# danielreardon/scintools

Hardware: NVIDIA H100
Metric: theta-theta eta-trials/sec on 4096x8192 dynspec (higher is better)
Workload: dtype f32

## Files before the change

### scintools_b200/csrc/thth.cu

```cuda
#include <float.h>
#include <limits.h>
#include <math.h>
#include <stdlib.h>

#include <type_traits>

#include "bf16_pack.cuh"
#include "lanczos.cuh"
#include "thth.cuh"
#include "tma.cuh"

namespace sb {

#ifndef SB_HOST_EMU
int eig_cluster_launch(const float2* d_M, int ld, int n_max, const int* d_nred, int e0,
                       int nb, double* d_eigs, int* d_status, int* d_iters, double tol,
                       double etol, int max_iter, cudaStream_t st);

int eig_half_launch(const float2* d_M, const unsigned* d_Mb, int ld, const int* d_nred, int e0,
                    int nb, double* d_eigs, int* d_status, int* d_iters, double tol, double etol,
                    int max_iter, bool tensor, cudaStream_t st);

#endif

enum { ST_OK = 0, ST_INDEX_ERROR = 1, ST_ZERO_START = 2, ST_TOO_SMALL = 4,
       ST_NOT_CONVERGED = 8 };

__global__ void thth_prep_kernel(ThthGeom g, const double* __restrict__ etas,
                                 int neta, int ld, int* __restrict__ idx,
                                 int* __restrict__ nred) {
    int e = blockIdx.x;
    if (e >= neta) return;
    double eta = etas[e];
    int lane = threadIdx.x;
    int base = 0;
    int* out = idx + (size_t)e * ld;
    for (int k0 = 0; k0 < g.n; k0 += 32) {
        int k = k0 + lane;
        bool keep = false;
        if (k < g.n) {
            double t = g.th[k];
            keep = (__dmul_rn(__dmul_rn(t, t), eta) < g.tau_absmax) &&
                   (fabs(t) < g.fd_half);
        }
        unsigned m = __ballot_sync(0xffffffffu, keep);
        if (keep) out[base + __popc(m & ((1u << lane) - 1u))] = k;
        base += __popc(m);
    }
    if (lane == 0) nred[e] = base;
}

__global__ void thth_indexerr_kernel(ThthGeom g, const double* __restrict__ etas,
                                     int* __restrict__ status) {
    int e = blockIdx.y;
    double eta = etas[e];
    long long total = (long long)g.n * g.n;
    bool bad = false;
    for (long long p = (long long)blockIdx.x * blockDim.x + threadIdx.x;
         p < total; p += (long long)gridDim.x * blockDim.x) {
        int i = (int)(p / g.n), j = (int)(p % g.n);
        ThthPoint pt = thth_point(g, eta, g.th[j], g.th[i]);
        bad |= pt.index_error;
    }
    if (__any_sync(0xffffffffu, bad) && (threadIdx.x & 31) == 0)
        atomicOr(status + e, ST_INDEX_ERROR);
}

#define SB_BUILD_EB 8

__device__ __forceinline__ unsigned pack_f16x2(float2 v) {
#ifdef SB_HOST_EMU
    const __half2 h = __floats2half2_rn(v.x, v.y);
    return (unsigned)h.x | ((unsigned)h.y << 16);
#else
    unsigned r;
    asm("cvt.rn.f16x2.f32 %0, %1, %2;" : "=r"(r) : "f"(v.y), "f"(v.x));
    return r;
#endif
}

__global__ void cs_absmax_kernel(const float2* __restrict__ cs, long long rows, long long ncols,
                                 long long pitch, unsigned* __restrict__ out) {
    float m = 0.f;
    const long long per_row4 = ncols >> 1;
    const long long total = rows * per_row4;
    for (long long i = (long long)blockIdx.x * blockDim.x + threadIdx.x; i < total;
         i += (long long)gridDim.x * blockDim.x) {
        const long long r = i / per_row4, c = i - r * per_row4;
        const float4 q = __ldg(reinterpret_cast<const float4*>(cs + r * pitch) + c);
        m = fmaxf(fmaxf(fmaxf(fabsf(q.x), fabsf(q.y)), fmaxf(fabsf(q.z), fabsf(q.w))), m);
    }
    if (ncols & 1) {
        for (long long r = (long long)blockIdx.x * blockDim.x + threadIdx.x; r < rows;
             r += (long long)gridDim.x * blockDim.x) {
            const float2 q = __ldg(cs + r * pitch + ncols - 1);
            m = fmaxf(fmaxf(fabsf(q.x), fabsf(q.y)), m);
        }
    }
    if (!(m == m)) m = 3.0e38f;
    m = fminf(m, 3.0e38f);
#pragma unroll
    for (int o = 16; o > 0; o >>= 1) m = fmaxf(m, __shfl_xor_sync(0xffffffffu, m, o));
    if ((threadIdx.x & 31) == 0) atomicMax(out, __float_as_uint(m));
}

template <int PACK, int ROWS, typename OFF>
__global__ void __launch_bounds__(32 * (32 / ROWS), ROWS == 8 ? 5 : 3)
thth_build_kernel(ThthGeom g, const double* __restrict__ etas, int eta0, int nbatch,
                  int ld, const int* __restrict__ idx,
                  const int* __restrict__ nred, float2* __restrict__ M,
                  unsigned* __restrict__ Mb, const unsigned* __restrict__ absmax, float span) {
    constexpr int TY = 32 / ROWS;
    int p = blockIdx.y, ta = 0;
    const int T = ld / 32;
    while (p >= T - ta) { p -= T - ta; ++ta; }
    const int tb = ta + p;
    const int tx = threadIdx.x, ty = threadIdx.y;
    const int b = tb * 32 + tx;
    const double ntau_d = (double)g.ntau;
    const long long hfd = g.nfd / 2;
    int cj = -2;
    double thj = 0.0;
    int ci[ROWS];
    double dk[ROWS];
    int col[ROWS];
    unsigned conj = 0u;
    float wk[ROWS];
#pragma unroll
    for (int k = 0; k < ROWS; ++k) { ci[k] = -2; dk[k] = 0.0; col[k] = -1; wk[k] = 0.f; }
    const int e_end = min(nbatch, (int)(blockIdx.x + 1) * SB_BUILD_EB);
    __shared__ float s_hscale[SB_BUILD_EB];
    if (PACK != 0) {
        const int lin = ty * 32 + tx;
        if (lin < SB_BUILD_EB) {
            const int e = blockIdx.x * SB_BUILD_EB + lin;
            float hs = 1.f;
            if (e < e_end) {
                const float seta = sqrtf((float)(2.0 * etas[eta0 + e]));
                const float bound = __uint_as_float(*absmax) * seta * sqrtf(span);
                if (bound > 0.f && bound < 3.0e38f) {
                    const float q = 32768.f / bound;
                    hs = q >= 1.1754944e-38f ? __uint_as_float(__float_as_uint(q) & 0x7f800000u) : 1.1754944e-38f;
                }
            }
            s_hscale[lin] = hs;
        }
        __syncthreads();
    }
    const unsigned foff0 = (unsigned)(ta * 32 + ty) * (unsigned)ld + (unsigned)b;
    const unsigned frow = (unsigned)TY * (unsigned)ld;
    const unsigned woff0 = ((unsigned)(2 * ta) * (unsigned)(ld >> 3) + (unsigned)(b >> 3)) * 128u +
                           (unsigned)ty * 8u;
    for (int e = blockIdx.x * SB_BUILD_EB; e < e_end; ++e) {
        const int n = nred[eta0 + e];
        if (tb * 32 >= n) continue;
        const double eta = etas[eta0 + e];
        const int* id = idx + (size_t)(eta0 + e) * ld;
        const int j = b < n ? id[b] : -1;
        if (j != cj) {
            cj = j;
            thj = j >= 0 ? g.th[j] : 0.0;
#pragma unroll
            for (int k = 0; k < ROWS; ++k) ci[k] = -2;
        }
        const float seta = sqrtf((float)(2.0 * eta));
        float2* Me = M + (size_t)e * ld * ld;
        const float hscale = PACK != 0 ? s_hscale[e - blockIdx.x * SB_BUILD_EB] : 1.f;
        OFF off[ROWS];
        unsigned hit = 0u;
#pragma unroll
        for (int k = 0; k < ROWS; ++k) {
            const int la = ty + TY * k;
            off[k] = 0;
            if (ta == tb && tx < la) continue;
            const int a = ta * 32 + la;
            const int i = a < n ? id[a] : -1;
            if (i != ci[k]) {
                ci[k] = i;
                col[k] = -1;
                conj &= ~(1u << k);
                wk[k] = 0.f;
                dk[k] = 0.0;
                if (i >= 0 && j > i && i + j != g.n - 1) {
                    const double th1 = thj, th2 = g.th[i];
                    dk[k] = __dsub_rn(__dmul_rn(th1, th1), __dmul_rn(th2, th2));
                    const double bb = __dadd_rn(__dsub_rn(__dsub_rn(th1, th2), g.fd0), g.half_dfd);
                    const double fqd = floor_div_fast(bb, g.dfd, g.inv_dfd);
                    const long long fq = (fqd == fqd && fabs(fqd) < 9.0e18) ? (long long)fqd : LLONG_MIN;
                    wk[k] = sqrtf((float)fabs(th2 - th1));
                    if (fq < g.nfd && !(fq < -g.nfd)) {
                        const long long fi = fq < 0 ? fq + g.nfd : fq;
                        if (!g.cs_half) col[k] = (int)fi;
                        else if (fi >= hfd) col[k] = (int)(fi - hfd);
                        else if (fi == 0) col[k] = (int)hfd;
                        else { col[k] = (int)(hfd - fi); conj |= 1u << k; }
                    }
                }
            }
            if (col[k] >= 0) {
                const double aa = __dadd_rn(__dsub_rn(__dmul_rn(eta, dk[k]), g.tau0), g.half_dtau);
                const double tqd = floor_div_fast(aa, g.dtau, g.inv_dtau);
                if (tqd > 0.0 && tqd < ntau_d) {
                    const int tq = (int)tqd;
                    const int r = (conj >> k) & 1u ? (int)g.ntau - tq : tq;
                    off[k] = (OFF)r * (OFF)g.cs_pitch + (OFF)col[k];
                    hit |= 1u << k;
                }
            }
        }
        float2 val[ROWS];
#pragma unroll
        for (int k = 0; k < ROWS; ++k) val[k] = __ldg(g.cs + off[k]);
#pragma unroll
        for (int k = 0; k < ROWS; ++k) {
            const int la = ty + TY * k;
            const bool low = ta == tb && tx < la;
            float2 v = make_float2(0.f, 0.f);
            if (!low) {
                if (col[k] >= 0) {
                    if ((hit >> k) & 1u) {
                        v = val[k];
                        if ((conj >> k) & 1u) v.y = -v.y;
                        if (!g.coherent) v = make_float2(hypotf(v.x, v.y), 0.f);
                    }
                    const float wf = seta * wk[k];
                    v.x *= wf;
                    v.y *= wf;
                    if (!(fabsf(v.x) <= 3.402823466e+38f) || !(fabsf(v.y) <= 3.402823466e+38f)) {
                        v.x = nan_to_num(v.x);
                        v.y = nan_to_num(v.y);
                    }
                }
                const unsigned o = foff0 + (unsigned)k * frow;
                Me[o] = v;
                if (PACK == 1) Mb[(size_t)e * ld * ld + o] = pack_f16x2(make_float2(v.x * hscale, v.y * hscale));
            }
            if (PACK == 2) {
                const unsigned h = low ? 0u : pack_f16x2(make_float2(v.x * hscale, v.y * hscale));
                const int i8 = tx & 7, s0 = (tx & ~7) + 2 * (i8 & 3);
                const unsigned ha = __shfl_sync(0xffffffffu, h, s0);
                const unsigned hb = __shfl_sync(0xffffffffu, h, s0 + 1);
                const unsigned word = i8 < 4 ? ((ha & 0xffffu) | (hb << 16)) : ((ha >> 16) | (hb & 0xffff0000u));
                if (!(ta == tb && (tx >> 4) < (la >> 4))) {
                    unsigned* Mw = Mb + (size_t)e * ld * ld;
                    const unsigned swz = (unsigned)(((la & 15) >> 2) & 1) << 2;
                    Mw[woff0 + (unsigned)(la >> 4) * (unsigned)(ld >> 3) * 128u + (unsigned)((la & 15) - ty) * 8u +
                       ((unsigned)i8 ^ swz)] = word;
                }
            }
        }
    }
}

template <int THREADS, bool TMA, int NST, bool FAST = false>
__global__ void __launch_bounds__(THREADS)
thth_eig_kernel(const float2* __restrict__ Mbase, int ld,
                const int* __restrict__ nred, int eta0,
                double* __restrict__ eigs, int* __restrict__ status,
                int* __restrict__ iters, double tol, double etol, int max_iter, int nb) {
    extern __shared__ __align__(128) unsigned char smem_raw[];
    constexpr int NW = THREADS / 32;
    LanczosShared& S = *reinterpret_cast<LanczosShared*>(smem_raw);
    float2* v = reinterpret_cast<float2*>(smem_raw + sizeof(LanczosShared));
    float2* vp = v + ld;
    float2* w = vp + ld;
    float2* u = w + ld;
    float4* stages = reinterpret_cast<float4*>(u + ld);
    float2* part = reinterpret_cast<float2*>(stages);
    unsigned long long* mbar = reinterpret_cast<unsigned long long*>(
        reinterpret_cast<unsigned char*>(stages) +
        (TMA ? (size_t)NW * NST * 4096 : (size_t)NW * 4096));
    const int tid = threadIdx.x, lane = tid & 31, warp = tid >> 5;
    if (TMA) {
        if (tid == 0) {
            for (int i = 0; i < NW * NST; ++i) mbar_init(mbar + i, 1);
            fence_mbarrier_init();
        }
    }
    unsigned gi = 0, gc = 0;
    for (int e = blockIdx.x; e < nb; e += gridDim.x) {
    __syncthreads();
    const int n = nred[eta0 + e];
    const float2* M = Mbase + (size_t)e * ld * ld;
    const double qnan = __longlong_as_double(0x7ff8000000000000LL);

    if (status[eta0 + e] & ST_INDEX_ERROR) {
        if (tid == 0) { eigs[eta0 + e] = qnan; iters[eta0 + e] = 0; }
        continue;
    }
    if (n < 3) {
        if (tid == 0) {
            eigs[eta0 + e] = qnan; iters[eta0 + e] = 0;
            status[eta0 + e] |= ST_TOO_SMALL;
        }
        continue;
    }
    const int h = n / 2;
    double part0 = 0.0;
    for (int c = tid; c < ld; c += THREADS) {
        float2 x = make_float2(0.f, 0.f);
        if (c < n && c > h) x = M[(size_t)h * ld + c];
        else if (c < h) { x = M[(size_t)c * ld + h]; x.y = -x.y; }
        v[c] = x;
        vp[c] = make_float2(0.f, 0.f);
        part0 += (double)x.x * x.x + (double)x.y * x.y;
    }
    part0 = warp_sum(part0);
    if (lane == 0) S.red[0][warp] = part0;
    if (tid == 0) {
        S.done = 0; S.lo = 0.0; S.theta = 0.0; S.res = 0.0; S.m_lo2 = 0; S.lo2 = 0.0;
        S.next_check = 1; S.m_last = 0; S.beta2[0] = 0.0;
    }
    __syncthreads();
    double nrm2 = 0.0;
    for (int k = 0; k < NW; ++k) nrm2 += S.red[0][k];
    if (!(nrm2 > 0.0) || !isfinite(nrm2)) {
        if (tid == 0) {
            eigs[eta0 + e] = qnan; iters[eta0 + e] = 0;
            status[eta0 + e] |= ST_ZERO_START;
        }
        continue;
    }
    {
        float s = (float)(1.0 / sqrt(nrm2));
        for (int c = tid; c < ld; c += THREADS) { v[c].x *= s; v[c].y *= s; }
    }
    __syncthreads();

    const int ncol4 = (n + 1) >> 1;
    const int nchunk = (n + 511) / 512;
    float4* mystage = stages + (size_t)warp * NST * 256;
    unsigned long long* mybar = mbar + warp * NST;
    float beta_prev = 0.f;
    int m = 0;
    for (int it = 0; it < max_iter; ++it) {
        for (int c = tid; c < ld; c += THREADS) w[c] = make_float2(0.f, 0.f);
        __syncthreads();
        if constexpr (TMA) {
            float4 yc[8];
#pragma unroll
            for (int j = 0; j < 8; ++j) yc[j] = make_float4(0.f, 0.f, 0.f, 0.f);
            const int K = (n - 2 >= warp) ? (n - 2 - warp) / NW + 1 : 0;
            const bool tail = ncol4 < 256;
            const float4* v4 = reinterpret_cast<const float4*>(v);
            for (int k = 0; k < NST && k < K; ++k) {
                const int st = gi % NST;
                ++gi;
                if (lane == 0) {
                    const int a = warp + NW * k;
                    const int c_lo = (a + 1) & ~1;
                    const unsigned bytes = (unsigned)(2 * ncol4 - c_lo) * 8u;
                    mbar_expect_tx(mybar + st, bytes);
                    bulk_g2s(reinterpret_cast<float2*>(mystage + st * 256) + c_lo,
                             M + (size_t)a * ld + c_lo, bytes, mybar + st);
                }
            }
            int k = 0;
            auto run_rows = [&](auto JSc) {
                constexpr int JS = decltype(JSc)::value;
                for (; k < K && ((warp + NW * k + 1) >> 6) == JS; ++k) {
                    const int a = warp + NW * k;
                    const int first4 = (a + 1) >> 1;
                    const float2 xa = v[a];
                    const int st = gc % NST;
                    const unsigned par = (gc / NST) & 1u;
                    ++gc;
                    while (!mbar_try_wait(mybar + st, par)) {}
                    const float4* sg = mystage + st * 256;
                    float rxa = 0.f, rxb = 0.f, rya = 0.f, ryb = 0.f;
#pragma unroll
                    for (int j = JS; j < 8; ++j) {
                        const int c4 = lane + 32 * j;
                        float4 q = sg[c4];
                        bool ok = (j > JS) || (c4 >= first4);
                        if (tail) ok = ok && (c4 < ncol4);
                        if (!ok) q = make_float4(0.f, 0.f, 0.f, 0.f);
                        float4 x = make_float4(0.f, 0.f, 0.f, 0.f);
                        if (ok) x = v4[c4];
                        rxa = fmaf(q.x, x.x, rxa); rxb = fmaf(-q.y, x.y, rxb);
                        rxa = fmaf(q.z, x.z, rxa); rxb = fmaf(-q.w, x.w, rxb);
                        rya = fmaf(q.x, x.y, rya); ryb = fmaf(q.y, x.x, ryb);
                        rya = fmaf(q.z, x.w, rya); ryb = fmaf(q.w, x.z, ryb);
                        yc[j].x = fmaf(q.x, xa.x, yc[j].x); yc[j].x = fmaf(q.y, xa.y, yc[j].x);
                        yc[j].y = fmaf(q.x, xa.y, yc[j].y); yc[j].y = fmaf(-q.y, xa.x, yc[j].y);
                        yc[j].z = fmaf(q.z, xa.x, yc[j].z); yc[j].z = fmaf(q.w, xa.y, yc[j].z);
                        yc[j].w = fmaf(q.z, xa.y, yc[j].w); yc[j].w = fmaf(-q.w, xa.x, yc[j].w);
                    }
                    __syncwarp();
                    const bool more = k + NST < K;
                    const int st2 = gi % NST;
                    if (more) ++gi;
                    if (lane == 0 && more) {
                        const int a2 = warp + NW * (k + NST);
                        const int c_lo = (a2 + 1) & ~1;
                        const unsigned bytes = (unsigned)(2 * ncol4 - c_lo) * 8u;
                        mbar_expect_tx(mybar + st2, bytes);
                        bulk_g2s(reinterpret_cast<float2*>(mystage + st2 * 256) + c_lo,
                                 M + (size_t)a2 * ld + c_lo, bytes, mybar + st2);
                    }
                    const float rx = rxa + rxb, ry = rya + ryb;
                    const bool hi = lane & 16;
                    float keep = hi ? ry : rx;
                    keep += __shfl_xor_sync(0xffffffffu, hi ? rx : ry, 16);
                    keep += __shfl_xor_sync(0xffffffffu, keep, 8);
                    keep += __shfl_xor_sync(0xffffffffu, keep, 4);
                    keep += __shfl_xor_sync(0xffffffffu, keep, 2);
                    keep += __shfl_xor_sync(0xffffffffu, keep, 1);
                    if (lane == 0) w[a].x += keep;
                    if (lane == 16) w[a].y += keep;
                }
            };
            run_rows(std::integral_constant<int, 0>{});
            run_rows(std::integral_constant<int, 1>{});
            run_rows(std::integral_constant<int, 2>{});
            run_rows(std::integral_constant<int, 3>{});
            run_rows(std::integral_constant<int, 4>{});
            run_rows(std::integral_constant<int, 5>{});
            run_rows(std::integral_constant<int, 6>{});
            run_rows(std::integral_constant<int, 7>{});
            __syncthreads();
#pragma unroll
            for (int j = 0; j < 8; ++j)
                *reinterpret_cast<float4*>(part + warp * 512 + 2 * (lane + 32 * j)) = yc[j];
            __syncthreads();
            for (int c = tid; c < 512; c += THREADS) {
                float sx = 0.f, sy = 0.f;
#pragma unroll
                for (int kk = 0; kk < NW; ++kk) { sx += part[kk * 512 + c].x; sy += part[kk * 512 + c].y; }
                if (c < ld) u[c] = make_float2(sx, sy);
            }
            fence_proxy_async();
            __syncthreads();
        } else {
        for (int cb = 0; cb < nchunk; ++cb) {
            float4 yc[8];
#pragma unroll
            for (int j = 0; j < 8; ++j) yc[j] = make_float4(0.f, 0.f, 0.f, 0.f);
            const int chunk_end = min(n, (cb + 1) * 512);
            const int K = (chunk_end - 2 >= warp) ? (chunk_end - 2 - warp) / NW + 1 : 0;
            if (TMA) {
                for (int k = 0; k < NST && k < K; ++k) {
                    const int st = gi % NST;
                    ++gi;
                    if (lane == 0) {
                        const int a = warp + NW * k;
                        const int c_lo = (a + 1) & ~1;
                        const unsigned bytes = (unsigned)(2 * ncol4 - c_lo) * 8u;
                        mbar_expect_tx(mybar + st, bytes);
                        bulk_g2s(reinterpret_cast<float2*>(mystage + st * 256) + c_lo,
                                 M + (size_t)a * ld + c_lo, bytes, mybar + st);
                    }
                }
            }
            for (int k = 0; k < K; ++k) {
                const int a = warp + NW * k;
                const int first4 = (a + 1) >> 1;
                const float2 xa = v[a];
                float4 mm[8];
                if (TMA) {
                    const int st = gc % NST;
                    const unsigned par = (gc / NST) & 1u;
                    ++gc;
                    while (!mbar_try_wait(mybar + st, par)) {}
                    const float4* sg = mystage + st * 256;
                    const int jlo = max(0, (first4 - lane + 31) >> 5);
                    const int jhi = (ncol4 - lane + 31) >> 5;
#pragma unroll
                    for (int j = 0; j < 8; ++j)
                        mm[j] = (j >= jlo && j < jhi) ? sg[lane + 32 * j]
                                                      : make_float4(0.f, 0.f, 0.f, 0.f);
                } else {
                    const float4* row = reinterpret_cast<const float4*>(M + (size_t)a * ld);
#pragma unroll
                    for (int j = 0; j < 8; ++j) {
                        const int c4 = cb * 256 + lane + 32 * j;
                        mm[j] = (c4 >= first4 && c4 < ncol4) ? __ldg(row + c4)
                                                             : make_float4(0.f, 0.f, 0.f, 0.f);
                    }
                }
                float rx = 0.f, ry = 0.f;
                const int jskip = (first4 - cb * 256) >> 5;
#pragma unroll
                for (int j = 0; j < 8; ++j) {
                    if (j < jskip) continue;
                    const int c4 = cb * 256 + lane + 32 * j;
                    const float4 q = mm[j];
                    const float4 x = (2 * c4 < ld) ? *reinterpret_cast<const float4*>(v + 2 * c4)
                                                   : make_float4(0.f, 0.f, 0.f, 0.f);
                    rx = fmaf(q.x, x.x, rx); rx = fmaf(-q.y, x.y, rx);
                    rx = fmaf(q.z, x.z, rx); rx = fmaf(-q.w, x.w, rx);
                    ry = fmaf(q.x, x.y, ry); ry = fmaf(q.y, x.x, ry);
                    ry = fmaf(q.z, x.w, ry); ry = fmaf(q.w, x.z, ry);
                    yc[j].x = fmaf(q.x, xa.x, yc[j].x); yc[j].x = fmaf(q.y, xa.y, yc[j].x);
                    yc[j].y = fmaf(q.x, xa.y, yc[j].y); yc[j].y = fmaf(-q.y, xa.x, yc[j].y);
                    yc[j].z = fmaf(q.z, xa.x, yc[j].z); yc[j].z = fmaf(q.w, xa.y, yc[j].z);
                    yc[j].w = fmaf(q.z, xa.y, yc[j].w); yc[j].w = fmaf(-q.w, xa.x, yc[j].w);
                }
                if (TMA) {
                    __syncwarp();
                    const bool more = k + NST < K;
                    const int st = gi % NST;
                    if (more) ++gi;
                    if (lane == 0 && more) {
                        const int a2 = warp + NW * (k + NST);
                        const int c_lo = (a2 + 1) & ~1;
                        const unsigned bytes = (unsigned)(2 * ncol4 - c_lo) * 8u;
                        mbar_expect_tx(mybar + st, bytes);
                        bulk_g2s(reinterpret_cast<float2*>(mystage + st * 256) + c_lo,
                                 M + (size_t)a2 * ld + c_lo, bytes, mybar + st);
                    }
                }
                rx = warp_sum(rx);
                ry = warp_sum(ry);
                if (lane == 0) { w[a].x += rx; w[a].y += ry; }
            }
            if (TMA) __syncthreads();
#pragma unroll
            for (int j = 0; j < 8; ++j)
                *reinterpret_cast<float4*>(part + warp * 512 + 2 * (lane + 32 * j)) = yc[j];
            __syncthreads();
            for (int c = tid; c < 512; c += THREADS) {
                float sx = 0.f, sy = 0.f;
#pragma unroll
                for (int k = 0; k < NW; ++k) { sx += part[k * 512 + c].x; sy += part[k * 512 + c].y; }
                if (cb * 512 + c < ld) u[cb * 512 + c] = make_float2(sx, sy);
            }
            if (TMA) fence_proxy_async();
            __syncthreads();
        }
        }
        double apart = 0.0;
        for (int c = tid; c < n; c += THREADS) {
            float2 x = w[c];
            x.x += u[c].x;
            x.y += u[c].y;
            w[c] = x;
            apart += (double)(v[c].x * x.x + v[c].y * x.y);
        }
        apart = warp_sum(apart);
        if (lane == 0) S.red[0][warp] = apart;
        __syncthreads();
        double alpha = 0.0;
        for (int k = 0; k < NW; ++k) alpha += S.red[0][k];
        const float af = (float)alpha;
        double bpart = 0.0;
        for (int c = tid; c < n; c += THREADS) {
            float2 x = w[c];
            x.x -= af * v[c].x + beta_prev * vp[c].x;
            x.y -= af * v[c].y + beta_prev * vp[c].y;
            w[c] = x;
            bpart += (double)x.x * x.x + (double)x.y * x.y;
        }
        bpart = warp_sum(bpart);
        if (lane == 0) S.red[1][warp] = bpart;
        __syncthreads();
        double b2 = 0.0;
        for (int k = 0; k < NW; ++k) b2 += S.red[1][k];
        const double beta = sqrt(b2);
        m = it + 1;
        if (tid == 0) { S.alpha[it] = alpha; S.beta[m] = beta; S.beta2[m] = b2; }
        __syncthreads();
        const bool last = (it + 1 == max_iter);
        if (warp == 0 && (m >= S.next_check || last || !(beta > 0.0))) {
            if (FAST) lanczos_check_fast(S, m, tol, etol);
            else lanczos_check(S, m, tol, etol);
        }
        __syncthreads();
        if (S.done || !isfinite(alpha)) break;
        const float ib = (float)(1.0 / beta);
        for (int c = tid; c < n; c += THREADS) {
            float2 x = w[c];
            vp[c] = v[c];
            v[c] = make_float2(x.x * ib, x.y * ib);
        }
        beta_prev = (float)beta;
        __syncthreads();
    }
    if (tid == 0) {
        eigs[eta0 + e] = fabs(S.theta);
        iters[eta0 + e] = m;
        if (!S.done) status[eta0 + e] |= ST_NOT_CONVERGED;
    }
    }
}

__global__ void thth_map_kernel(ThthGeom g, double eta, int hermitian,
                                float2* __restrict__ out,
                                int* __restrict__ tau_inv,
                                int* __restrict__ fd_inv,
                                unsigned char* __restrict__ pnts,
                                int* __restrict__ err) {
    long long total = (long long)g.n * g.n;
    for (long long p = (long long)blockIdx.x * blockDim.x + threadIdx.x;
         p < total; p += (long long)gridDim.x * blockDim.x) {
        int i = (int)(p / g.n), j = (int)(p % g.n);
        double thi = g.th[i], thj = g.th[j];
        ThthPoint pt = thth_point(g, eta, thj, thi);
        if (pt.index_error) atomicOr(err, ST_INDEX_ERROR);
        if (tau_inv) tau_inv[p] = (int)max(min(pt.tq, (long long)INT_MAX), (long long)INT_MIN);
        if (fd_inv) fd_inv[p] = (int)max(min(pt.fq, (long long)INT_MAX), (long long)INT_MIN);
        if (pnts) pnts[p] = pt.pnt ? 1 : 0;
        if (!out) continue;
        float2 v;
        if (!hermitian) {
            v = thth_value(g, eta, thj, thi, pt);
        } else if (i == j || i + j == g.n - 1) {
            v = make_float2(0.f, 0.f);
        } else if (j > i) {
            v = thth_value(g, eta, thj, thi, pt);
            v.x = nan_to_num(v.x);
            v.y = nan_to_num(v.y);
        } else {
            ThthPoint pu = thth_point(g, eta, thi, thj);
            v = thth_value(g, eta, thi, thj, pu);
            v.x = nan_to_num(v.x);
            v.y = -nan_to_num(v.y);
        }
        out[p] = v;
    }
}

#ifndef SB_HOST_EMU
static bool lower_check_needed(const ThthGeom& g, const double* th_host) {
    double tmin = th_host[0], tmax = th_host[0];
    for (int k = 1; k < g.n; ++k) {
        tmin = th_host[k] < tmin ? th_host[k] : tmin;
        tmax = th_host[k] > tmax ? th_host[k] : tmax;
    }
    double worst = floor(((tmin - tmax) - g.fd0 + g.half_dfd) / g.dfd) - 2.0;
    return !(worst >= -(double)g.nfd);
}

int eta_sweep(const ThthGeom& g, const double* th_host, const double* d_etas,
              int neta, double tol, int max_iter, double* d_eigs,
              int* d_status, int* d_nred, int* d_iters, cudaStream_t st) {
    if (neta <= 0) return SB_OK;
    if (max_iter <= 0 || max_iter > SB_LANCZOS_MAXIT) max_iter = SB_LANCZOS_MAXIT;
    const int ld = (g.n + 31) / 32 * 32;
    if (ld > 4096) {
        set_error("theta-theta grid of %d centres exceeds the supported 4096", g.n);
        return SB_ERR_UNSUPPORTED;
    }
    int* d_idx = (int*)workspace(1, (size_t)neta * ld * sizeof(int));
    if (!d_idx) return SB_ERR_NOMEM;
    SB_CUDA(cudaMemsetAsync(d_status, 0, neta * sizeof(int), st));
    prof_begin(PROF_THTH_PREP, st);
    thth_prep_kernel<<<neta, 32, 0, st>>>(g, d_etas, neta, ld, d_idx, d_nred);
    prof_end(PROF_THTH_PREP, st);
    SB_LAUNCH_CHECK();
    if (lower_check_needed(g, th_host)) {
        dim3 grid(64, neta);
        thth_indexerr_kernel<<<grid, 256, 0, st>>>(g, d_etas, d_status);
        SB_LAUNCH_CHECK();
    }
    const size_t per = (size_t)ld * ld * sizeof(float2);
    unsigned long long slab = 3ull << 30;
    if (const char* ev = getenv("SB_SWEEP_SLAB_MB")) {
        const long mb = atol(ev);
        if (mb > 0) slab = (unsigned long long)mb << 20;
    }
    int batch = (int)(slab / per);
    if (batch < 1) batch = 1;
    if (batch > neta) batch = neta;
    float2* d_M = (float2*)workspace(2, per * batch);
    if (!d_M) return SB_ERR_NOMEM;
    const bool mixed = (ld <= 512) && !getenv("SB_EIG_FP32") && !getenv("SB_EIG_CLUSTER") &&
                       !getenv("SB_EIG_PERSIST") && !getenv("SB_EIG_NO_TMA");
    unsigned* d_Mb = nullptr;
    if (mixed) {
        d_Mb = (unsigned*)workspace(6, per / 2 * batch);
        if (!d_Mb) return SB_ERR_NOMEM;
    }
    const int T = ld / 32;
    const int npairs = T * (T + 1) / 2;
    constexpr int TT = 256, TS = 2;
    constexpr int DT = 512;
    const bool use_tma = (ld <= 512) && !getenv("SB_EIG_NO_TMA");
    const size_t smem = sizeof(LanczosShared) + 4 * (size_t)ld * sizeof(float2) +
                        (use_tma ? (size_t)(TT / 32) * TS * 4096 + 512
                                 : (size_t)(DT / 32) * 4096 + 512);
    int persist = 0;
    if (const char* ev = getenv("SB_EIG_PERSIST")) persist = atoi(ev);
    constexpr int PS = 4;
    const size_t smem_p = sizeof(LanczosShared) + 4 * (size_t)ld * sizeof(float2) +
                          (size_t)(TT / 32) * PS * 4096 + 512;
    if (use_tma && persist > 0)
        SB_CUDA(cudaFuncSetAttribute(thth_eig_kernel<TT, true, PS, true>,
                                     cudaFuncAttributeMaxDynamicSharedMemorySize, (int)smem_p));
    if (use_tma)
        SB_CUDA(cudaFuncSetAttribute(thth_eig_kernel<TT, true, TS>,
                                     cudaFuncAttributeMaxDynamicSharedMemorySize, (int)smem));
    else
        SB_CUDA(cudaFuncSetAttribute(thth_eig_kernel<DT, false, 1>,
                                     cudaFuncAttributeMaxDynamicSharedMemorySize, (int)smem));
    unsigned* d_absmax = nullptr;
    float span = 0.f;
    if (mixed) {
        d_absmax = (unsigned*)workspace(0, 64 * sizeof(double)) + 32;
        if (!d_absmax) return SB_ERR_NOMEM;
        if (g.cs_bound) {
            SB_CUDA(cudaMemcpyAsync(d_absmax, g.cs_bound, sizeof(float), cudaMemcpyDeviceToDevice, st));
        } else {
            SB_CUDA(cudaMemsetAsync(d_absmax, 0, sizeof(unsigned), st));
            const long long ncols = g.cs_half ? (g.cs_valid_cols > 0 ? g.cs_valid_cols : g.nfd / 2 + 1)
                                              : g.nfd;
            cs_absmax_kernel<<<num_sms() * 8, 256, 0, st>>>(g.cs, g.ntau, ncols, g.cs_pitch, d_absmax);
            SB_LAUNCH_CHECK();
        }
        double tmin = th_host[0], tmax = th_host[0];
        for (int k = 1; k < g.n; ++k) {
            tmin = th_host[k] < tmin ? th_host[k] : tmin;
            tmax = th_host[k] > tmax ? th_host[k] : tmax;
        }
        span = (float)((tmax - tmin) * 1.0001);
    }
    for (int e0 = 0; e0 < neta; e0 += batch) {
        int nb = neta - e0 < batch ? neta - e0 : batch;
        static const int BR = (getenv("SB_BUILD_ROWS") && atoi(getenv("SB_BUILD_ROWS")) == 8) ? 8 : 4;
        const bool tensor = mixed && BR == 4 && !getenv("SB_EIG_NO_TC");
        dim3 grid((nb + SB_BUILD_EB - 1) / SB_BUILD_EB, npairs), block(32, 32 / BR);
        prof_begin(PROF_THTH_BUILD, st);
        const bool small = (unsigned long long)g.ntau * (unsigned long long)g.cs_pitch < (1ull << 32);
#define SB_BUILD_LAUNCH(PACK, ROWS, OFF, MB, AM, SP)                                        \
        thth_build_kernel<PACK, ROWS, OFF><<<grid, block, 0, st>>>(g, d_etas, e0, nb, ld, d_idx, \
                                                                   d_nred, d_M, MB, AM, SP)
        if (BR == 8) {
            if (mixed && small) SB_BUILD_LAUNCH(1, 8, unsigned, d_Mb, d_absmax, span);
            else if (mixed) SB_BUILD_LAUNCH(1, 8, size_t, d_Mb, d_absmax, span);
            else if (small) SB_BUILD_LAUNCH(0, 8, unsigned, nullptr, nullptr, 0.f);
            else SB_BUILD_LAUNCH(0, 8, size_t, nullptr, nullptr, 0.f);
        } else if (tensor) {
            if (small) SB_BUILD_LAUNCH(2, 4, unsigned, d_Mb, d_absmax, span);
            else SB_BUILD_LAUNCH(2, 4, size_t, d_Mb, d_absmax, span);
        } else {
            if (mixed && small) SB_BUILD_LAUNCH(1, 4, unsigned, d_Mb, d_absmax, span);
            else if (mixed) SB_BUILD_LAUNCH(1, 4, size_t, d_Mb, d_absmax, span);
            else if (small) SB_BUILD_LAUNCH(0, 4, unsigned, nullptr, nullptr, 0.f);
            else SB_BUILD_LAUNCH(0, 4, size_t, nullptr, nullptr, 0.f);
        }
#undef SB_BUILD_LAUNCH
        prof_end(PROF_THTH_BUILD, st);
        SB_LAUNCH_CHECK();
        prof_begin(PROF_THTH_EIG, st);
        int rc = mixed ? eig_half_launch(d_M, d_Mb, ld, d_nred, e0, nb, d_eigs, d_status,
                                         d_iters, tol, 2e-7, max_iter, tensor, st)
                       : 0;
        if (rc == 0)
            rc = eig_cluster_launch(d_M, ld, g.n, d_nred, e0, nb, d_eigs, d_status, d_iters,
                                    tol, 2e-7, max_iter, st);
        if (rc < 0) return rc;
        if (rc > 0) {
        } else if (use_tma && persist > 0)
            thth_eig_kernel<TT, true, PS, true><<<persist < nb ? persist : nb, TT, smem_p, st>>>(
                d_M, ld, d_nred, e0, d_eigs, d_status, d_iters, tol, 2e-7, max_iter, nb);
        else if (use_tma)
            thth_eig_kernel<TT, true, TS><<<nb, TT, smem, st>>>(
                d_M, ld, d_nred, e0, d_eigs, d_status, d_iters, tol, 2e-7, max_iter, nb);
        else
            thth_eig_kernel<DT, false, 1><<<nb, DT, smem, st>>>(
                d_M, ld, d_nred, e0, d_eigs, d_status, d_iters, tol, 2e-7, max_iter, nb);
        prof_end(PROF_THTH_EIG, st);
        SB_LAUNCH_CHECK();
    }
    return SB_OK;
}

__global__ void thth_mask_kernel(ThthGeom g, double eta,
                                 unsigned char* __restrict__ mask) {
    int k = blockIdx.x * blockDim.x + threadIdx.x;
    if (k >= g.n) return;
    double t = g.th[k];
    mask[k] = ((__dmul_rn(__dmul_rn(t, t), eta) < g.tau_absmax) &&
               (fabs(t) < g.fd_half)) ? 1 : 0;
}

int thth_map(const ThthGeom& g, double eta, int hermitian, float2* d_out,
             int* d_tau_inv, int* d_fd_inv, unsigned char* d_pnts,
             unsigned char* d_th_pnts, int* d_err, cudaStream_t st) {
    if (d_th_pnts) {
        thth_mask_kernel<<<(g.n + 255) / 256, 256, 0, st>>>(g, eta, d_th_pnts);
        SB_LAUNCH_CHECK();
    }
    if (!d_err) return SB_OK;
    SB_CUDA(cudaMemsetAsync(d_err, 0, sizeof(int), st));
    long long total = (long long)g.n * g.n;
    int blocks = (int)((total + 255) / 256);
    if (blocks > num_sms() * 16) blocks = num_sms() * 16;
    thth_map_kernel<<<blocks, 256, 0, st>>>(g, eta, hermitian, d_out, d_tau_inv,
                                            d_fd_inv, d_pnts, d_err);
    SB_LAUNCH_CHECK();
    return SB_OK;
}

#endif

}
```

Before: 122,900.

## Gather reached conjugate-spectrum columns into a compact column-major copy for build

Before the build loop, marks which conjugate-spectrum columns any theta pair can reach, prefix-sums them into compact slots, and transposes those columns into a contiguous column-major buffer indexed by delay. The build kernel then gathers from this compact buffer using slot*ntau+row offsets instead of the row-major pitched spectrum. The aim is better cache locality, since the gathers for a fixed column walk along delay, and a smaller working set. In exchange it adds three preprocessing kernels, one of them a single-block scan, plus an extra workspace buffer sized by a host-side bound on reachable columns.

After: 130,600, median of 6. 6.2% higher.

```diff
diff --git a/scintools_b200/csrc/thth.cu b/scintools_b200/csrc/thth.cu
--- a/scintools_b200/csrc/thth.cu
+++ b/scintools_b200/csrc/thth.cu
@@ -4,6 +4,11 @@
 #include <stdlib.h>
 
 #include <type_traits>
+#ifdef SB_HOST_EMU
+#include <cstdio>
+#include <cstdlib>
+#include <vector>
+#endif
 
 #include "bf16_pack.cuh"
 #include "lanczos.cuh"
@@ -66,6 +71,117 @@
         atomicOr(status + e, ST_INDEX_ERROR);
 }
 
+__device__ __forceinline__ int thth_sweep_column(const ThthGeom& g, double th1, double th2,
+                                                 bool* cj) {
+    const double bb = __dadd_rn(__dsub_rn(__dsub_rn(th1, th2), g.fd0), g.half_dfd);
+    const double fqd = floor_div_fast(bb, g.dfd, g.inv_dfd);
+    const long long fq = (fqd == fqd && fabs(fqd) < 9.0e18) ? (long long)fqd : LLONG_MIN;
+    *cj = false;
+    if (!(fq < g.nfd) || fq < -g.nfd) return -1;
+    const long long fi = fq < 0 ? fq + g.nfd : fq;
+    if (!g.cs_half) return (int)fi;
+    const long long hfd = g.nfd / 2;
+    if (fi >= hfd) return (int)(fi - hfd);
+    if (fi == 0) return (int)hfd;
+    *cj = true;
+    return (int)(hfd - fi);
+}
+
+__global__ void __launch_bounds__(256) thth_colmark_kernel(ThthGeom g, int* __restrict__ mark) {
+    const int i = blockIdx.y;
+    const int j = blockIdx.x * blockDim.x + threadIdx.x;
+    if (j <= i || j >= g.n || i + j == g.n - 1) return;
+    bool cj;
+    const int c = thth_sweep_column(g, g.th[j], g.th[i], &cj);
+    if (c >= 0) mark[c] = 1;
+}
+
+__global__ void __launch_bounds__(1024) thth_colslot_kernel(int ncols, const int* __restrict__ mark,
+                                                            int* __restrict__ colslot,
+                                                            int* __restrict__ slotcol,
+                                                            int* __restrict__ nslots) {
+    SB_SHARED int s_warp[32];
+    const int t = threadIdx.x, lane = t & 31, w = t >> 5, nw = blockDim.x >> 5;
+    const int per = (ncols + blockDim.x - 1) / blockDim.x;
+    const int c0 = min(ncols, t * per), c1 = min(ncols, c0 + per);
+    int cnt = 0;
+    for (int c = c0; c < c1; ++c) cnt += mark[c] != 0;
+    int inc = cnt;
+#pragma unroll
+    for (int o = 1; o < 32; o <<= 1) {
+        const int y = __shfl_sync(0xffffffffu, inc, lane - o);
+        if (lane >= o) inc += y;
+    }
+    if (lane == 31) s_warp[w] = inc;
+    __syncthreads();
+    int s = inc - cnt, total = 0;
+    for (int k = 0; k < nw; ++k) {
+        const int v = s_warp[k];
+        if (k < w) s += v;
+        total += v;
+    }
+    for (int c = c0; c < c1; ++c) {
+        if (mark[c]) {
+            colslot[c] = s;
+            slotcol[s++] = c;
+        } else {
+            colslot[c] = -1;
+        }
+    }
+    if (t == 0) *nslots = total;
+}
+
+__global__ void __launch_bounds__(256) thth_colcopy_kernel(ThthGeom g, const int* __restrict__ slotcol,
+                                                           const int* __restrict__ nslots,
+                                                           long long maxslots,
+                                                           float2* __restrict__ csc) {
+    SB_SHARED float2 tile[32][33];
+    const int ns = *nslots < maxslots ? *nslots : (int)maxslots;
+    const int tx = threadIdx.x, ty = threadIdx.y;
+    const long long ntau = g.ntau;
+    const long long rtiles = (ntau + 31) / 32;
+    const long long ntiles = rtiles * ((ns + 31) / 32);
+    for (long long tix = blockIdx.x; tix < ntiles; tix += gridDim.x) {
+        const int s0 = (int)(tix / rtiles) * 32;
+        const long long r0 = (tix % rtiles) * 32;
+        const int s = s0 + tx;
+        const long long c = s < ns ? slotcol[s] : 0;
+#pragma unroll
+        for (int k = 0; k < 4; ++k) {
+            const long long r = r0 + ty + 8 * k;
+            if (s < ns && r < ntau) tile[ty + 8 * k][tx] = __ldg(g.cs + r * g.cs_pitch + c);
+        }
+        __syncthreads();
+#pragma unroll
+        for (int k = 0; k < 4; ++k) {
+            const int so = s0 + ty + 8 * k;
+            const long long r = r0 + tx;
+            if (so < ns && r < ntau) csc[(size_t)so * (size_t)ntau + (size_t)r] = tile[tx][ty + 8 * k];
+        }
+        __syncthreads();
+    }
+}
+
+static long long reached_columns_bound(const ThthGeom& g, const double* th_host, long long ncols) {
+    if (g.n < 2) return 0;
+    double lo = th_host[0], hi = th_host[0];
+    double dmin = INFINITY, dmax = -INFINITY;
+    for (int j = 1; j < g.n; ++j) {
+        const double a = th_host[j] - hi, b = th_host[j] - lo;
+        dmin = a < dmin ? a : dmin;
+        dmax = b > dmax ? b : dmax;
+        lo = th_host[j] < lo ? th_host[j] : lo;
+        hi = th_host[j] > hi ? th_host[j] : hi;
+    }
+    long long bound = ncols;
+    const double qlo = floor((dmin - g.fd0 + g.half_dfd) / g.dfd);
+    const double qhi = floor((dmax - g.fd0 + g.half_dfd) / g.dfd);
+    const double span = qhi - qlo + 3.0;
+    if (span >= 0.0 && span < (double)bound) bound = (long long)span;
+    const long long npairs = (long long)g.n * (g.n - 1) / 2;
+    return bound < npairs ? bound : npairs;
+}
+
 #define SB_BUILD_EB 8
 
 __device__ __forceinline__ unsigned pack_f16x2(float2 v) {
@@ -106,7 +222,8 @@
 
 template <int PACK, int ROWS, typename OFF>
 __global__ void __launch_bounds__(32 * (32 / ROWS), ROWS == 8 ? 5 : 3)
-thth_build_kernel(ThthGeom g, const double* __restrict__ etas, int eta0, int nbatch,
+thth_build_kernel(ThthGeom g, const float2* __restrict__ csc, const int* __restrict__ colslot,
+                  const double* __restrict__ etas, int eta0, int nbatch,
                   int ld, const int* __restrict__ idx,
                   const int* __restrict__ nred, float2* __restrict__ M,
                   unsigned* __restrict__ Mb, const unsigned* __restrict__ absmax, float span) {
@@ -118,7 +235,6 @@
     const int tx = threadIdx.x, ty = threadIdx.y;
     const int b = tb * 32 + tx;
     const double ntau_d = (double)g.ntau;
-    const long long hfd = g.nfd / 2;
     int cj = -2;
     double thj = 0.0;
     int ci[ROWS];
@@ -184,16 +300,12 @@
                 if (i >= 0 && j > i && i + j != g.n - 1) {
                     const double th1 = thj, th2 = g.th[i];
                     dk[k] = __dsub_rn(__dmul_rn(th1, th1), __dmul_rn(th2, th2));
-                    const double bb = __dadd_rn(__dsub_rn(__dsub_rn(th1, th2), g.fd0), g.half_dfd);
-                    const double fqd = floor_div_fast(bb, g.dfd, g.inv_dfd);
-                    const long long fq = (fqd == fqd && fabs(fqd) < 9.0e18) ? (long long)fqd : LLONG_MIN;
                     wk[k] = sqrtf((float)fabs(th2 - th1));
-                    if (fq < g.nfd && !(fq < -g.nfd)) {
-                        const long long fi = fq < 0 ? fq + g.nfd : fq;
-                        if (!g.cs_half) col[k] = (int)fi;
-                        else if (fi >= hfd) col[k] = (int)(fi - hfd);
-                        else if (fi == 0) col[k] = (int)hfd;
-                        else { col[k] = (int)(hfd - fi); conj |= 1u << k; }
+                    bool cjk;
+                    const int c = thth_sweep_column(g, th1, th2, &cjk);
+                    if (c >= 0) {
+                        col[k] = colslot[c];
+                        if (cjk) conj |= 1u << k;
                     }
                 }
             }
@@ -203,14 +315,14 @@
                 if (tqd > 0.0 && tqd < ntau_d) {
                     const int tq = (int)tqd;
                     const int r = (conj >> k) & 1u ? (int)g.ntau - tq : tq;
-                    off[k] = (OFF)r * (OFF)g.cs_pitch + (OFF)col[k];
+                    off[k] = (OFF)col[k] * (OFF)g.ntau + (OFF)r;
                     hit |= 1u << k;
                 }
             }
         }
         float2 val[ROWS];
 #pragma unroll
-        for (int k = 0; k < ROWS; ++k) val[k] = __ldg(g.cs + off[k]);
+        for (int k = 0; k < ROWS; ++k) val[k] = __ldg(csc + off[k]);
 #pragma unroll
         for (int k = 0; k < ROWS; ++k) {
             const int la = ty + TY * k;
@@ -251,6 +363,47 @@
         }
     }
 }
+
+#ifdef SB_HOST_EMU
+struct EmuColumnCopy {
+    std::vector<int> colslot;
+    std::vector<float2> csc;
+};
+
+static void emu_column_copy(const ThthGeom& g, EmuColumnCopy& cc) {
+    const long long ncols = g.cs_half ? g.nfd / 2 + 1 : g.nfd;
+    std::vector<int> mark(ncols, 0);
+    for (int i = 0; i < g.n; ++i)
+        for (int j = i + 1; j < g.n; ++j) {
+            bool cj;
+            const int c = i + j == g.n - 1 ? -1 : thth_sweep_column(g, g.th[j], g.th[i], &cj);
+            if (c >= 0) mark[c] = 1;
+        }
+    const long long maxslots = reached_columns_bound(g, g.th, ncols);
+    cc.colslot.assign(ncols, -1);
+    cc.csc.assign((size_t)(maxslots > 0 ? maxslots : 1) * (size_t)g.ntau, make_float2(0.f, 0.f));
+    long long s = 0;
+    for (long long c = 0; c < ncols; ++c) {
+        if (!mark[c]) continue;
+        if (s >= maxslots) {
+            std::fprintf(stderr, "emu_column_copy: more reached columns than the bound %lld\n", maxslots);
+            std::abort();
+        }
+        cc.colslot[c] = (int)s;
+        for (long long r = 0; r < g.ntau; ++r) cc.csc[(size_t)s * g.ntau + r] = g.cs[r * g.cs_pitch + c];
+        ++s;
+    }
+}
+
+template <int PACK, int ROWS, typename OFF>
+void thth_build_kernel(ThthGeom g, const double* etas, int eta0, int nbatch, int ld, const int* idx,
+                       const int* nred, float2* M, unsigned* Mb, const unsigned* absmax, float span) {
+    static EmuColumnCopy cc;
+    if (threadIdx.x == 0 && threadIdx.y == 0) emu_column_copy(g, cc);
+    thth_build_kernel<PACK, ROWS, OFF>(g, cc.csc.data(), cc.colslot.data(), etas, eta0, nbatch, ld, idx,
+                                       nred, M, Mb, absmax, span);
+}
+#endif
 
 template <int THREADS, bool TMA, int NST, bool FAST = false>
 __global__ void __launch_bounds__(THREADS)
@@ -641,8 +794,17 @@
         set_error("theta-theta grid of %d centres exceeds the supported 4096", g.n);
         return SB_ERR_UNSUPPORTED;
     }
-    int* d_idx = (int*)workspace(1, (size_t)neta * ld * sizeof(int));
+    const long long ncols = g.cs_half ? g.nfd / 2 + 1 : g.nfd;
+    int* d_idx = (int*)workspace(1, ((size_t)neta * ld + 3 * (size_t)ncols + 1) * sizeof(int));
     if (!d_idx) return SB_ERR_NOMEM;
+    int* d_mark = d_idx + (size_t)neta * ld;
+    int* d_colslot = d_mark + ncols;
+    int* d_slotcol = d_colslot + ncols;
+    int* d_nslots = d_slotcol + ncols;
+    const long long maxslots = reached_columns_bound(g, th_host, ncols);
+    const size_t csc_elems = (size_t)(maxslots > 0 ? maxslots : 1) * (size_t)g.ntau;
+    float2* d_csc = (float2*)workspace(4, csc_elems * sizeof(float2));
+    if (!d_csc) return SB_ERR_NOMEM;
     SB_CUDA(cudaMemsetAsync(d_status, 0, neta * sizeof(int), st));
     prof_begin(PROF_THTH_PREP, st);
     thth_prep_kernel<<<neta, 32, 0, st>>>(g, d_etas, neta, ld, d_idx, d_nred);
@@ -714,16 +876,26 @@
         }
         span = (float)((tmax - tmin) * 1.0001);
     }
+    prof_begin(PROF_THTH_BUILD, st);
+    SB_CUDA(cudaMemsetAsync(d_mark, 0, (size_t)ncols * sizeof(int), st));
+    thth_colmark_kernel<<<dim3((g.n + 255) / 256, g.n > 0 ? g.n : 1), 256, 0, st>>>(g, d_mark);
+    SB_LAUNCH_CHECK();
+    thth_colslot_kernel<<<1, 1024, 0, st>>>((int)ncols, d_mark, d_colslot, d_slotcol, d_nslots);
+    SB_LAUNCH_CHECK();
+    thth_colcopy_kernel<<<num_sms() * 8, dim3(32, 8), 0, st>>>(g, d_slotcol, d_nslots, maxslots, d_csc);
+    prof_end(PROF_THTH_BUILD, st);
+    SB_LAUNCH_CHECK();
     for (int e0 = 0; e0 < neta; e0 += batch) {
         int nb = neta - e0 < batch ? neta - e0 : batch;
         static const int BR = (getenv("SB_BUILD_ROWS") && atoi(getenv("SB_BUILD_ROWS")) == 8) ? 8 : 4;
         const bool tensor = mixed && BR == 4 && !getenv("SB_EIG_NO_TC");
         dim3 grid((nb + SB_BUILD_EB - 1) / SB_BUILD_EB, npairs), block(32, 32 / BR);
         prof_begin(PROF_THTH_BUILD, st);
-        const bool small = (unsigned long long)g.ntau * (unsigned long long)g.cs_pitch < (1ull << 32);
+        const bool small = csc_elems < (1ull << 32);
 #define SB_BUILD_LAUNCH(PACK, ROWS, OFF, MB, AM, SP)                                        \
-        thth_build_kernel<PACK, ROWS, OFF><<<grid, block, 0, st>>>(g, d_etas, e0, nb, ld, d_idx, \
-                                                                   d_nred, d_M, MB, AM, SP)
+        thth_build_kernel<PACK, ROWS, OFF><<<grid, block, 0, st>>>(g, d_csc, d_colslot, d_etas, e0, \
+                                                                   nb, ld, d_idx, d_nred, d_M, MB, \
+                                                                   AM, SP)
         if (BR == 8) {
             if (mixed && small) SB_BUILD_LAUNCH(1, 8, unsigned, d_Mb, d_absmax, span);
             else if (mixed) SB_BUILD_LAUNCH(1, 8, size_t, d_Mb, d_absmax, span);
```
